# sMedX/FaceNet

Hardware: AMD Instinct MI355X
Metric: images/sec (160x160 triplet train) (higher is better)
Workload: dtype bf16

## Files before the change

### facenet_amd/_lib.py

```python
from __future__ import annotations

import ctypes as C
import os

import torch

_HERE = os.path.dirname(os.path.abspath(__file__))
LIB_PATH = os.path.join(_HERE, "lib", "libfacenet_hip.so")

FN_BF16, FN_F16 = 0, 1
FN_OPT_ADAGRAD, FN_OPT_ADADELTA, FN_OPT_RMSPROP, FN_OPT_MOM = 1, 2, 3, 4


class ConvDesc(C.Structure):
    _fields_ = [
        ("N", C.c_int32), ("H", C.c_int32), ("W", C.c_int32), ("Cin", C.c_int32),
        ("OH", C.c_int32), ("OW", C.c_int32), ("Cout", C.c_int32),
        ("KH", C.c_int32), ("KW", C.c_int32), ("stride", C.c_int32), ("pad_h", C.c_int32), ("pad_w", C.c_int32),
        ("dtype", C.c_int32), ("ld_x", C.c_int32), ("ld_y", C.c_int32),
        ("relu", C.c_int32), ("accumulate", C.c_int32), ("out_f32", C.c_int32), ("ld_res", C.c_int32),
        ("scale", C.c_float), ("splits", C.c_int32), ("stats_sq_off", C.c_int32), ("stats_replicas", C.c_int32),
        ("stats_rep_stride", C.c_int32),
        ("x", C.c_void_p), ("w", C.c_void_p), ("y", C.c_void_p), ("dx", C.c_void_p), ("dw", C.c_void_p),
        ("bias", C.c_void_p), ("stats", C.c_void_p), ("resid", C.c_void_p),
# ... 11 lines not shown

class FacenetHipError(RuntimeError):
    pass


_i, _f, _p, _l, _u = C.c_int, C.c_float, C.c_void_p, C.c_long, C.c_uint32

_SIGNATURES = {
    "fn_abi_version": [],
    "fn_conv2d_fwd": [C.POINTER(ConvDesc), _p],
    "fn_conv2d_dgrad": [C.POINTER(ConvDesc), _p],
    "fn_conv2d_wgrad": [C.POINTER(ConvDesc), _p],
    "fn_conv2d_variant": [C.POINTER(ConvDesc), _i],
    "fn_block35_infer": [_p, _p, _i, _p, _p, _p, _p, _p, _p, _f, _i, _i, _p],
    "fn_block35_infer_warm": [_p, _p, _i, _p, _p, _p, _p, _p, _p, _f, _i, _p, C.c_int64, _i, _p],
    "fn_block17_infer": [_p, _p, _i, _p, _p, _p, _p, _p, _p, _p, _p, _p, _p, _f, _i, _i, _p],
    "fn_block17_infer_warm": [_p, _p, _i, _p, _p, _p, _p, _p, _p, _p, _p, _p, _p, _f, _i, _p, C.c_int64, _i, _p],
    "fn_conv2d_arg_bytes": [],
    "fn_conv2d_group_build": [C.POINTER(ConvDesc), _i, _i, _i, _p, _p, _p],
    "fn_conv2d_grouped": [_p, _p, _i, _i, _i, _i, _i, _i, _p],
    "fn_conv2d_wgrad_arg_bytes": [],
    "fn_conv2d_wgrad_group_build": [C.POINTER(ConvDesc), _i, _i, _p, _p, _p, _p],
    "fn_conv2d_wgrad_reduce": [_p, _i, _p],
    "fn_conv2d_wgrad_grouped": [_p, _p, _i, _i, _i, _i, _p],
    "fn_image_normalize": [_p, _p, _p, _i, _i, _i, _i, _p],
    "fn_image_normalize_f32": [_p, _p, _p, _i, _i, _i, _i, _p],
    "fn_image_resize_bilinear": [_p, _i, _p, _i, _i, _i, _i, _i, _p],
    "fn_bn_finalize": [_p, _i, _i, _p, _p, _p, _p, _p, _p, _p, _f, _f, _i, _p],
    "fn_crop_or_pad_u8": [_p, _p, _p, _p, _i, _i, _p],
    "fn_augment_u8": [_p, _p, _p, _p, _p, _i, _i, _p],
    "fn_gather_images": [_p, _p, _p, _i, _i, _p],
    "fn_bn_relu_train_fwd": [_p, _i, _p, _i, _i, _i, _p, _i, _i, _i, _p, _p, _p, _p, _p, _f, _f, _i, _i, _p],
    "fn_bn_relu_train_bwd": [_p, _i, _p, _i, _i, _i, _p, _p, _p, _p, _p, _i, _i, _i, _i, _i, _i, _p],
    "fn_maxpool3x3s2_fwd": [_p, _i, _p, _i, _i, _i, _i, _i, _p, _i, _p],
    "fn_maxpool3x3s2_bwd": [_p, _i, _p, _i, _p, _i, _i, _i, _i, _i, _p, _i, _i, _p],
    "fn_area_resize_crop": [_p, _i, _i, _p, _i, _i, _i, _i, _p, _i, _p],
    "fn_maxpool2d_fwd": [_p, _i, _p, _i, _i, _i, _i, _i, _i, _i, _i, _i, _i, _i, _i, _p],
    "fn_area_resize_frame": [_p, _i, _i, _i, _i, _p, _p, _i, _p],
    "fn_mtcnn_candidates": [_p, C.c_long, _i, _f, _p, _p, _i, _i, _i, _p],
    "fn_nms_greedy_batch": [_p, _i, _p, _p, _p, _p, _i, _p, C.c_long, _p, _p, _p],
    "fn_nms_greedy": [_p, _i, _p, _i, C.c_double, _i, _p, C.c_long, _p, _p, _p],
    "fn_avgpool_fwd": [_p, _p, _i, _i, _i, _i, _p],
    "fn_avgpool_bwd": [_p, _p, _i, _i, _i, _i, _p],
    "fn_avgpool3x3s1_fwd": [_p, _i, _p, _i, _i, _i, _i, _i, _i, _p],
    "fn_avgpool3x3s1_bwd": [_p, _i, _p, _i, _i, _i, _i, _i, _i, _i, _p],
    "fn_dropout_fwd": [_p, _p, _i, _i, _f, _u, _i, _p, _i, _p],
    "fn_dropout_bwd": [_p, _p, _i, _i, _f, _u, _i, _p, _i, _p],
    "fn_residual_bwd": [_p, _p, _p, _p, _p, _i, _i, _f, _i, _i, _i, _p],
    "fn_acc_to_float": [_p, _p, _l, _i, _p],
    "fn_head_bn_fwd": [_p, _p, _i, _i, _p, _p, _p, _p, _p, _i, _f, _f, _p],
    "fn_head_bn_bwd": [_p, _p, _p, _p, _p, _p, _i, _i, _i, _p],
    "fn_l2norm_fwd": [_p, _p, _i, _i, _f, _p],
    "fn_l2norm_bwd": [_p, _p, _p, _i, _i, _f, _p],
    "fn_cast_f32_to_lp": [_p, _p, _l, _i, _p],
    "fn_pairwise_sqdist": [_p, _p, _p, _p, _i, _i, _i, _i, _p],
    "fn_select_triplets": [_p, _p, _i, _f, _i, _u, _i, _p, _p, _p],
    "fn_triplet_loss_fwd_bwd": [_p, _p, _p, _i, _i, _f, _p],
    "fn_confidence_counts": [_p, _p, _i, _i, _p, _i, _i, _p, _p, _p],
    "fn_confidence_counts_folds": [_p, _p, _p, _p, _p, _i, _i, _i, _p, _i, _i, _p, _p, _p],
    "fn_softmax_xent_fwd_bwd": [_p, _i, _p, _p, _p, _i, _p, _i, _i, _f, _i, _p],
    "fn_center_loss_fwd_bwd": [_p, _p, _p, _p, _p, _p, _i, _i, _i, _i, _f, _f, _f, _p],
    "fn_center_update": [_p, _i, _i, _i, _p, _i, C.c_double, _p],
    "fn_f2f_row_norms": [_p, _i, _i, _p, _p],
    "fn_f2f_pair_loss_fwd_bwd": [_p, _p, _i, _p, _i, _i, _i, _i, _f, _p, _p, _p, _p, _l, _p],
    "fn_f2f_pair_counts": [_p, _p, _p, _i, _i, _i, _p, _p, _p],
    "fn_f2f_distance": [_p, _p, _i, _p, _p, _i, _i, _i, _p, _i, _p, _p],
    "fn_adam_keras":[_p, _p, _p, _p, _p, _l, _l, _l, _p, _f, _f, _f, _f, _i, _p],
    "fn_adam_keras_ema": [_p, _p, _p, _p, _p, _l, _l, _l, _p, _f, _f, _f, _f, _i, _p, _f, _p],
    "fn_adam_tick": [_p, _f, _f, _p],
    "fn_opt_keras": [_i, _p, _p, _p, _p, _p, _l, _l, _l, _p, _f, _f, _f, _f, _i, _p],
    "fn_opt_keras_ema": [_i, _p, _p, _p, _p, _p, _l, _l, _l, _p, _f, _f, _f, _f, _i, _p, _f, _p],
    "fn_pack_transpose": [_p, _p, _p, _i, _i, _i, _p],
# ... 44 lines not shown
```

### facenet_amd/csrc/common.h

```cpp
#pragma once
#include <hip/hip_runtime.h>
#include <stdint.h>
#include <atomic>

namespace fn {

enum { FN_OK = 0, FN_EINVAL = -1, FN_ELAUNCH = -2, FN_EUNSUPPORTED = -3 };
void set_error(const char* fmt, ...);
int check_launch(const char* what);

#define FN_REQUIRE(cond, ...)                  \
    do {                                       \
        if (!(cond)) {                         \
            fn::set_error(__VA_ARGS__);        \
            return fn::FN_EINVAL;              \
        }                                      \
    } while (0)

typedef __attribute__((ext_vector_type(8))) __bf16 bf16x8;
typedef __attribute__((ext_vector_type(4))) __bf16 bf16x4;
typedef __attribute__((ext_vector_type(8))) _Float16 f16x8;
typedef __attribute__((ext_vector_type(4))) _Float16 f16x4;
typedef __attribute__((ext_vector_type(4))) float f32x4;
typedef __attribute__((ext_vector_type(4))) short s16x4;
// ... 90 lines not shown
    const float a = moving * momentum, w = 1.f - momentum;
    const float b = batch * w;
    return a + b;
}

__device__ __forceinline__ void bn_batch_affine(const acc_t* __restrict__ stats, int c, int sq_off, int reps, int rep_stride, int count,
                                                float eps, float beta, float& scale, float& shift, float& mean, float& var) {
    acc_t s = 0, q = 0;
    for (int rp = 0; rp < reps; ++rp) {
        s += stats[(long)rp * rep_stride + c];
        q += stats[(long)rp * rep_stride + sq_off + c];
    }
    bn_affine_from_sums(acc_get<ACC_STAT>(s), acc_get<ACC_STAT>(q), count, eps, beta, scale, shift, mean, var);
}

enum { STORE_WT = 17 };
__device__ __forceinline__ __amdgpu_buffer_rsrc_t wt_rsrc(const void* base) {
    return __builtin_amdgcn_make_buffer_rsrc(const_cast<void*>(base), 0, 0x7fffffff, 0x00020000);
}
__device__ __forceinline__ void store_wt(const __amdgpu_buffer_rsrc_t rs, long byte_offset, u32x4 v) {
    __builtin_amdgcn_raw_buffer_store_b128(v, rs, (int)byte_offset, 0, STORE_WT);
}

__device__ __forceinline__ int xcd_remap(int bid, int nwg) {
    const int q = nwg >> 3, r = nwg & 7, x = bid & 7;
    const int base = (x < r) ? x * (q + 1) : r * (q + 1) + (x - r) * q;
    return base + (bid >> 3);
}

static inline int cdiv(long a, long b) { return (int)((a + b - 1) / b); }

struct LdsOptIn {
    std::atomic<bool> done[32];
};
static inline int allow_big_lds(const void* kernel, LdsOptIn& state, const char* what) {
    int dev = 0;
    if (hipGetDevice(&dev) != hipSuccess || dev < 0 || dev >= 32) {
        set_error("%s: no current HIP device (or more than 32 devices)", what);
        return FN_ELAUNCH;
    }
    if (state.done[dev].load(std::memory_order_relaxed)) return FN_OK;
    const hipError_t e = hipFuncSetAttribute(kernel, hipFuncAttributeMaxDynamicSharedMemorySize, 160 * 1024);
    if (e != hipSuccess) {
        set_error("%s: hipFuncSetAttribute(MaxDynamicSharedMemorySize, 160 KiB) failed on device %d: %s", what, dev, hipGetErrorString(e));
        return FN_ELAUNCH;
    }
    state.done[dev].store(true, std::memory_order_relaxed);
// ... 12 lines not shown
```

### facenet_amd/csrc/conv_igemm.hip

```cpp
#include "common.h"
#include "../../include/facenet_hip.h"
#include "wgrad_taps.h"
#include <cstdio>
#include <type_traits>
#include <cstdlib>

#ifndef FN_IG_DBG
#define FN_IG_DBG 0
#endif

#if FN_IG_DBG & 32
__device__ unsigned long long fn_ig_phase[256 * 576 * 16];
extern "C" int fn_debug_phases(unsigned long long* out, int reset) {
    static unsigned long long host[256 * 576 * 16];
    if (out) {
        if (hipMemcpyFromSymbol(host, HIP_SYMBOL(fn_ig_phase), sizeof(host)) != hipSuccess) return -1;
        for (int i = 0; i < 576 * 16; ++i) {
            out[i] = 0;
            for (int r = 0; r < 256; ++r) out[i] += host[r * 576 * 16 + i];
        }
    }
    if (reset) {
        for (auto& v : host) v = 0;
        if (hipMemcpyToSymbol(HIP_SYMBOL(fn_ig_phase), host, sizeof(host)) != hipSuccess) return -1;
// ... 1173 lines not shown
    FN_REQUIRE(d->Cin % 8 == 0, "conv: Cin=%d must be a multiple of 8 (pad the input channels)", d->Cin);
    FN_REQUIRE(d->ld_x % 8 == 0 && d->ld_x >= d->Cin, "conv: ld_x=%d invalid for Cin=%d", d->ld_x, d->Cin);
    FN_REQUIRE(d->stride == 1 || d->stride == 2, "conv: stride %d unsupported", d->stride);
    FN_REQUIRE(d->KH >= 1 && d->KW >= 1 && d->KH < 256 && d->KW < 256, "conv: kernel %dx%d unsupported", d->KH, d->KW);
    FN_REQUIRE(d->N > 0 && d->H > 0 && d->W > 0 && d->OH > 0 && d->OW > 0 && d->Cout > 0, "conv: empty geometry");
    FN_REQUIRE((d->H + 2 * d->pad_h - d->KH) / d->stride + 1 == d->OH && (d->W + 2 * d->pad_w - d->KW) / d->stride + 1 == d->OW,
               "conv: OHxOW=%dx%d inconsistent with HxW=%dx%d k=%dx%d s=%d pad=%d,%d", d->OH, d->OW, d->H, d->W, d->KH, d->KW,
               d->stride, d->pad_h, d->pad_w);
    FN_REQUIRE((long)d->N * d->H * d->W < (1L << 31) / 8 && (long)d->N * d->OH * d->OW < (1L << 24) * 8L,
               "conv: tensor too large for 32-bit pixel indexing");
    return FN_OK;
}

struct WgradArgs {
    WgradOut out;
    const unsigned short* x;
    const unsigned short* dy;
    float* dw;
    int M, OH, OW, H, W, Cin, Cout, KTOT, KW;
    int stride, pad_h, pad_w;
    int ld_x, ld_y;
    int chunk;
    int gx, gy, splits;
    int plain;
    float inv_ow, inv_ohw;
    int x_bytes, dy_bytes;
    const acc_t* nrm_stats;
    const float* nrm_beta;
    int nrm_sq_off, nrm_replicas, nrm_rep_stride, nrm_count;
    float nrm_eps;
};

template <typename T, int BMW, int BNW, bool NORM>
__device__ __forceinline__ void conv_wgrad_body(const WgradArgs& a, const int bx, const int by, const int bz) {
    constexpr int BK = 64;
    constexpr int DEPTH = (BMW * BNW <= 64 * 64) ? 3 : (BMW * BNW <= 64 * 128 ? 2 : 1);
    constexpr int RSA = BMW * 2 + 32;
    constexpr int RSB = BNW * 2 + 32;
    constexpr int A_BYTES = BK * RSA, B_BYTES = BK * RSB;
    constexpr int CGA = BMW / 8, CGB = BNW / 8;
    constexpr int AP = BK * CGA / 256, BP = BK * CGB / 256;
    constexpr int WMW = (BMW >= 64) ? 2 : 1, WNW = 4 / WMW;
    constexpr int TM = BMW / WMW, TN = BNW / WNW;
    constexpr int MREP = TM / 16, NREP = TN / 16;
    static_assert(AP >= 1 && BP >= 1 && MREP >= 1 && NREP >= 1, "tile too small");
    typedef typename LP<T>::vec8 vec8;
// ... 185 lines not shown
    const long n4 = (long)a.Cout * a.KTOT / 4;
    const f32x4* ws = reinterpret_cast<const f32x4*>(a.ws);
    f32x4* dw = reinterpret_cast<f32x4*>(a.dw);
    for (long i = (long)blockIdx.x * 256 + threadIdx.x; i < n4; i += (long)gridDim.x * 256) {
        f32x4 s = ws[i];
        int z = 1;
        for (; z + 8 <= a.splits; z += 8) {
            f32x4 v[8];
#pragma unroll
            for (int k = 0; k < 8; ++k) v[k] = ws[(long)(z + k) * n4 + i];
#pragma unroll
            for (int k = 0; k < 8; ++k) s += v[k];
        }
        for (; z < a.splits; ++z) s += ws[(long)z * n4 + i];
        dw[i] = s;
    }
}

template <typename T, int BMW, int BNW, bool NORM>
__global__ __launch_bounds__(256) void conv_wgrad_kernel(const WgradArgs a) {
    conv_wgrad_body<T, BMW, BNW, NORM>(a, blockIdx.x, blockIdx.y, blockIdx.z);
}

template <typename T, int BMW, int BNW, bool NORM>
__global__ __launch_bounds__(256) void conv_wgrad_grouped_kernel(const unsigned char* __restrict__ args_raw, int stride, const int* __restrict__ prefix, int n) {
    const int bid = blockIdx.x;
    int lo = 0, hi = n;
    while (hi - lo > 1) {
        const int mid = (lo + hi) >> 1;
        if (prefix[mid] <= bid) lo = mid; else hi = mid;
    }
    lo = __builtin_amdgcn_readfirstlane(lo);
    const WgradArgs a = *reinterpret_cast<const WgradArgs*>(args_raw + (long)lo * stride);
    const int gxy = a.gx * a.gy;
    const int local = xcd_remap(bid - prefix[lo], gxy * a.splits);
    const int bz = local / gxy, r = local - bz * gxy;
    conv_wgrad_body<T, BMW, BNW, NORM>(a, r % a.gx, r / a.gx, bz);
}

template <typename T, int BMW, int BNW> static int launch_wgrad(const WgradArgs& a, int splits, hipStream_t st) {
    constexpr int RSA = BMW * 2 + 32, RSB = BNW * 2 + 32;
    const size_t smem = 2 * 64 * (RSA + RSB) + (a.nrm_stats ? 2 * BNW * 4 : 0);
    dim3 grid(cdiv(a.KTOT, BNW), cdiv(a.Cout, BMW), splits);
    if (a.nrm_stats) hipLaunchKernelGGL((conv_wgrad_kernel<T, BMW, BNW, true>), grid, dim3(256), smem, st, a);
    else hipLaunchKernelGGL((conv_wgrad_kernel<T, BMW, BNW, false>), grid, dim3(256), smem, st, a);
    return check_launch("conv_wgrad");
}

static void choose_wgrad_tile(int Cout, int KTOT, int& bmw, int& bnw) {
    bmw = Cout <= 32 ? 32 : (Cout <= 64 || Cout % 128 != 0 ? 64 : 128);
    bnw = (KTOT <= 64 || (cdiv(KTOT, 128) * 128 - KTOT) > 32) ? 64 : 128;
}

static int choose_wgrad_splits(int M, int Cout, int KTOT, int bmw, int bnw) {
    const long tiles = (long)cdiv(KTOT, bnw) * cdiv(Cout, bmw);
    const int stages = cdiv(M, 64);
    static const int stem_wgs = getenv("FN_WG_STEMWGS") ? atoi(getenv("FN_WG_STEMWGS")) : 1024;
    if (stages >= 1024) {
        int s = (int)((stem_wgs + tiles - 1) / tiles);
        if (s > stages / 4) s = stages / 4;
// ... 273 lines not shown
    long total = 0;
    for (int i = 0; i < n; ++i) {
        WgradArgs a;
        if (int rc = make_wgrad_args(&descs[i], a)) return rc;
        int m, k;
        final_wgrad_tile(a.Cout, a.KTOT, m, k);
        FN_REQUIRE(m == bmw && k == bnw, "wgrad_group_build: descriptor %d dispatches to %dx%d, group is %dx%d", i, m, k, bmw, bnw);
        FN_REQUIRE(descs[i].dtype == descs[0].dtype, "wgrad_group_build: mixed dtypes");
        FN_REQUIRE((a.nrm_stats != nullptr) == norm, "wgrad_group_build: descriptor %d: normalise-on-load members need a group of their own (variant + 1000000)", i);
        const int splits = plan_wgrad(a, descs[i].splits, bmw, bnw, true);
        FN_REQUIRE(((long)a.Cout * a.KTOT) % 4 == 0, "wgrad_group_build: descriptor %d: Cout*K must be a multiple of 4", i);
        a.out = WgradOut{a.dw, nullptr, a.Cout, a.KTOT, splits, 1};
        if (splits > 1) {
            a.out.ws = ws ? ws + ws_used : reinterpret_cast<float*>(16);
            ws_used += (long)splits * a.Cout * a.KTOT;
        }
        host_prefix[i] = (int32_t)total;
        total += (long)a.gx * a.gy * splits;
        *reinterpret_cast<WgradArgs*>(reinterpret_cast<unsigned char*>(host_args) + i * rec_bytes) = a;
    }
    FN_REQUIRE(total < (1L << 30), "wgrad_group_build: too many workgroups");
    host_prefix[n] = (int32_t)total;
    *ws_elems = ws_used;
    return (int)total;
}

extern "C" int fn_conv2d_wgrad_reduce(const void* dev_args, int n, void* stream) {
    FN_REQUIRE(dev_args && n > 0 && n < 65536, "wgrad_reduce: bad arguments");
    hipLaunchKernelGGL(wgrad_reduce_kernel, dim3(64, n), dim3(256), 0, (hipStream_t)stream, reinterpret_cast<const unsigned char*>(dev_args),
                       fn_conv2d_wgrad_arg_bytes());
    return check_launch("wgrad_reduce");
}

template <typename T> static int launch_wgrad_grouped(const void* args, const int32_t* prefix, int n, int total, int variant, hipStream_t st) {
    const bool norm = variant >= 1000000;
    variant %= 1000000;
    const int bmw = variant / 1000, bnw = variant % 1000;
    const unsigned char* a = reinterpret_cast<const unsigned char*>(args);
    const int stride_ = fn_conv2d_wgrad_arg_bytes();
#define FN_WG(BM_, BN_)                                                                                                     \
    if (bmw == BM_ && bnw == BN_) {                                                                                         \
        const size_t sm_ = 2 * 64 * ((BM_) * 2 + 32 + (BN_) * 2 + 32) + (norm ? 2 * (BN_) * 4 : 0);                            \
        if (norm) hipLaunchKernelGGL((conv_wgrad_grouped_kernel<T, BM_, BN_, true>), dim3(total), dim3(256), sm_, st, a, stride_, prefix, n); \
        else hipLaunchKernelGGL((conv_wgrad_grouped_kernel<T, BM_, BN_, false>), dim3(total), dim3(256), sm_, st, a, stride_, prefix, n);    \
        return check_launch("conv_wgrad_grouped");                                                                          \
    }
    FN_WG(32, 64) FN_WG(32, 128) FN_WG(64, 64) FN_WG(64, 128) FN_WG(128, 64) FN_WG(128, 128)
// ... 35 lines not shown
```

### facenet_amd/csrc/elementwise.hip

```cpp
#include "common.h"
#include "../../include/facenet_hip.h"

namespace fn {

__device__ __forceinline__ unsigned f2ord(float f) {
    unsigned u = __float_as_uint(f);
    return (u & 0x80000000u) ? ~u : (u | 0x80000000u);
}
__device__ __forceinline__ float ord2f(unsigned u) {
    return __uint_as_float((u & 0x80000000u) ? (u & 0x7fffffffu) : ~u);
}

template <typename SRC>
__global__ __launch_bounds__(256) void img_stats_kernel(const SRC* __restrict__ img, unsigned* __restrict__ work, int count) {
    const int n = blockIdx.y;
    const SRC* p = img + (long)n * count;
    float mx = -3e38f, mn = 3e38f, s = 0.f, q = 0.f;
    constexpr int PER = 16 / sizeof(SRC);
    const int head = min(count, (int)(((16 - ((uintptr_t)p & 15)) & 15) / sizeof(SRC)));
    const int nvec = (count - head) / PER;
    const SRC* pv = p + head;
    for (int i = blockIdx.x * 256 + threadIdx.x; i < nvec; i += gridDim.x * 256) {
        const u32x4 v = *reinterpret_cast<const u32x4*>(pv + (long)i * PER);
#pragma unroll
// ... 968 lines not shown
extern "C" int fn_l2norm_bwd(const float* x, const float* dout, float* dx, int N, int E, float eps, void* stream) {
    FN_REQUIRE(x && dout && dx && N > 0 && E > 0, "l2norm_bwd: bad arguments");
    hipLaunchKernelGGL(l2norm_bwd_kernel, dim3(cdiv(N, 4)), dim3(256), 0, (hipStream_t)stream, x, dout, dx, N, E, eps);
    return check_launch("l2norm_bwd");
}
extern "C" int fn_cast_f32_to_lp(const float* x, void* y, long n, int dtype, void* stream) {
    DT_CHECK(dtype);
    FN_REQUIRE(x && y && n > 0, "cast: bad arguments");
    LAUNCH_T(dtype, cast_kernel, dim3(grid_for(n)), dim3(256), 0, (hipStream_t)stream, x, (unsigned short*)y, n);
    return check_launch("cast");
}

namespace fn {
__global__ __launch_bounds__(256) void acc_to_float_kernel(const acc_t* __restrict__ src, float* __restrict__ dst, long n, double scale) {
    for (long i = (long)blockIdx.x * 256 + threadIdx.x; i < n; i += (long)gridDim.x * 256) dst[i] = (float)((double)src[i] * scale);
}
}
extern "C" int fn_acc_to_float(const fn_acc_t* src, float* dst, long n, int bits, void* stream) {
    FN_REQUIRE(src && dst && n > 0 && bits >= 0 && bits < 63, "acc_to_float: bad arguments");
    hipLaunchKernelGGL(acc_to_float_kernel, dim3(grid_for(n)), dim3(256), 0, (hipStream_t)stream, reinterpret_cast<const acc_t*>(src), dst, n,
                       1.0 / (double)(1ll << bits));
    return check_launch("acc_to_float");
}
```

### facenet_amd/train.py

```python
from __future__ import annotations

import contextlib
import ctypes as C
import json
import os
import warnings
from typing import Callable, Dict, List, NamedTuple, Optional, Sequence, Tuple

import numpy as np
import torch

from . import _lib, parallel
from .config import Config
from .engine import BN_EPS, L2_WEIGHT, Lowering, Network, _pad8, _ptr
from .schedule import Op, Schedule, StreamSet, levelize, make_events, region, run_schedule, torch_op


class GraphRunner:

    def __init__(self, device: torch.device):
        self.device = device
        self.graphs: List[torch.cuda.CUDAGraph] = []
        self.pool = None

    def capture(self, fn: Callable[[], None]) -> torch.cuda.CUDAGraph:
        g = torch.cuda.CUDAGraph()
        with torch.cuda.graph(g, pool=self.pool):
            fn()
        if self.pool is None:
            self.pool = g.pool()
        self.graphs.append(g)
        return g


def group_wgrads(ops: List[Op], net: Network) -> List[Op]:
    lib = net.lib
    singles = [op for op in ops if op.name.startswith("conv_wgrad:") and op.keep]
    if len(singles) < 2:
        return list(ops)
    rest = [op for op in ops if not (op.name.startswith("conv_wgrad:") and op.keep)]
    groups = {}
    for op in singles:
        d = op.keep[0]
        v = lib.fn_conv2d_variant(C.byref(d), 2)
        groups.setdefault((v + (1000000 if d.nrm_stats and v < 5000000 else 0), d.dtype), []).append(op)
    nbytes = lib.fn_conv2d_wgrad_arg_bytes()
    out = list(rest)
    split_tables, split_keep, split_writes = [], [], []
    for (variant, dt), members in sorted(groups.items()):
        n = len(members)
        descs = (_lib.ConvDesc * n)(*[m.keep[0] for m in members])
        host_args = (C.c_uint8 * (nbytes * n))()
        host_prefix = (C.c_int32 * (n + 1))()
        ws_elems = C.c_int64(0)
        total = lib.fn_conv2d_wgrad_group_build(descs, n, variant, host_args, host_prefix, None, C.byref(ws_elems))
        if total < 0:
            _lib.check(total, "wgrad_group_build")
        ws = torch.empty(max(1, ws_elems.value), dtype=torch.float32, device=net.device)
        total = lib.fn_conv2d_wgrad_group_build(descs, n, variant, host_args, host_prefix, _ptr(ws), C.byref(ws_elems))
        if total < 0:
            _lib.check(total, "wgrad_group_build")
        dev_args = torch.frombuffer(bytearray(host_args), dtype=torch.uint8).to(net.device)
        dev_prefix = torch.tensor(list(host_prefix), dtype=torch.int32, device=net.device)
        reads, writes = [], []
        for m in members:
            reads.extend(m.reads)
            writes.extend(m.writes)
        if variant >= 5000000:
            code = variant - 5000000
            name = f"conv_wgrad_taps:{code // 1000}x{code % 1000 // 10}" + ("s2" if code % 10 else "")
        else:
            name = f"conv_wgrad_grouped:{variant % 1000000 // 1000}x{variant % 1000}" + (":norm" if variant >= 1000000 else "")
# ... 230 lines not shown
        self.G = net.alloc_grads()
        self.slots: List[torch.Tensor] = [torch.full_like(self.G, init) for _, init in self.rule.slots]
        self.M, self.V = self.slots if self.optimizer == "ADAM" else (None, None)
        self.hyper = torch.tensor([lr, 1.0, 1.0, 1.0 / world_size, 0.0, 0.0, 0.0, 0.0], dtype=torch.float32, device=dev)
        self.loss = torch.zeros(4, dtype=torch.float32, device=dev)
        if world_size > 1:
            parallel.broadcast_parameters([net.P, net.S_mean, net.S_var], src=0, group=process_group)
            net.folded_valid = False
            net.refresh_packs()
        self.shadow: Optional[torch.Tensor] = None if self.ema_decay is None else net.P.clone()
        rank = 0
        if self.exchange:
            import torch.distributed as dist
            rank = dist.get_rank(process_group)
        self.rank = rank
        self.plan: Lowering = net.plan(batch, training=True, step_word=self.hyper.view(torch.int32)[4:5], rank=rank)
        self.demb = torch.zeros(batch, E, dtype=torch.float32, device=dev)
        self.dt = _lib.dtype_code(net.train_dtype)
        ebuf = self.plan.embedding.buf
        emb = ebuf.act
        r_emb = region(emb)
        self.emb = emb.view(batch, E)
        self.pre_ops: List[Op] = [
            Op("zero_grads", torch_op(lambda: (self.G.zero_(), net.Gacc.zero_())), (), writes=(region(self.G), region(net.Gacc))),
            Op("zero_bn_workspace", torch_op(lambda: (self.plan.ws.zero_(), self.plan.ws_b.zero_())), (),
               writes=(region(self.plan.ws), (self.plan.ws.data_ptr() + 1, 0, net.CB), region(self.plan.ws_b),
                       (self.plan.ws_b.data_ptr() + 1, 0, net.CB))),
        ]
        self.loss_ops: List[Op] = []
        if loss == "triplet":
            self.embn = torch.zeros(batch, E, dtype=torch.float32, device=dev)
            self.dembn = torch.zeros(batch, E, dtype=torch.float32, device=dev)
            self._op(self.loss_ops, "l2norm_fwd", lib.fn_l2norm_fwd, _ptr(emb), _ptr(self.embn), batch, E, 1e-10,
                     r=[r_emb], w=[region(self.embn)])
            self._op(self.loss_ops, "triplet_loss", lib.fn_triplet_loss_fwd_bwd, _ptr(self.embn), _ptr(self.dembn), _ptr(self.loss),
                     batch // 3, E, alpha, r=[region(self.embn)], w=[region(self.dembn), region(self.loss)])
            self._op(self.loss_ops, "l2norm_bwd", lib.fn_l2norm_bwd, _ptr(emb), _ptr(self.dembn), _ptr(self.demb), batch, E, 1e-10,
                     r=[r_emb, region(self.dembn)], w=[region(self.demb)])
        else:
            L = net.layers["classifier/logits"]
            Cp, Cr = L.cout, L.cout_real
            self.labels = torch.zeros(batch, dtype=torch.int32, device=dev)
            self.emb_lp = torch.zeros(batch, E, dtype=net.train_dtype, device=dev)
            self.logits = torch.zeros(batch, Cp, dtype=torch.float32, device=dev)
            self.dlogits = torch.zeros(batch, Cp, dtype=net.train_dtype, device=dev)
            rw = region(net.W_train, L.w_off, L.w_off + L.numel)
            rwt = region(net.Wt_train, L.w_off, L.w_off + L.numel)
            rgw = region(self.G, L.w_off, L.w_off + L.numel)
            rgb = region(net.Gacc, L.bias_off - net.bias_lo, L.bias_off - net.bias_lo + L.cout)
            d = self._cls_desc(L)
# ... 25 lines not shown
                        net.n_decay, _ptr(self.hyper), beta1, beta2, epsilon, l2, self.dt)
        else:
            rule = self.rule
            name, fn, fn_ema = rule.op, lib.fn_opt_keras, lib.fn_opt_keras_ema
            s2 = _ptr(self.slots[1]) if len(self.slots) > 1 else None
            opt_args = (rule.code, _ptr(net.P), _ptr(self.G), _ptr(self.slots[0]), s2, _ptr(net.W_train), net.n_kernel, net.n_params,
                        net.n_decay, _ptr(self.hyper), rule.rho, rule.momentum, rule.epsilon, l2, self.dt)
        if self.shadow is None:
            self._op(self.opt_ops, name, fn, *opt_args, r=[region(self.G), region(self.hyper)], w=opt_writes)
        else:
            self._op(self.opt_ops, name + "_ema", fn_ema, *opt_args, _ptr(self.shadow), self.ema_decay,
                     r=[region(self.G), region(self.hyper)], w=opt_writes + [region(self.shadow)])
        self._op(self.opt_ops, "pack_transpose", lib.fn_pack_transpose, _ptr(net.W_train), _ptr(net.Wt_train), _ptr(net.table),
                 len(net.layers), net.max_layer_elems, self.dt, r=[region(net.W_train)], w=[region(net.Wt_train)])
        if self.centers is not None:
            self._op(self.opt_ops, "center_update", lib.fn_center_update, _ptr(self.center_rows), E + 1, self.world * batch, E,
                     _ptr(self.centers), self.centers.shape[0], self.center_alfa, r=[region(self.center_rows)], w=[region(self.centers)])
        n_buckets = int(os.environ.get("FACENET_DP_BUCKETS", n_buckets))
        self.buckets = self._make_buckets(n_buckets) if self.segmented else []
        self.comm_stream = torch.cuda.Stream(device=dev) if self.exchange else None
        self.streams = _streams_for(net, n_streams)
        self.tiles = autotune_convs(self.plan.fwd + self.loss_ops + self.plan.bwd, net)
        self._build_segments()
        self._graph = None
        self._exchange_events: Optional[dict] = None
        self._eval_plans: Dict[int, Tuple[Lowering, torch.Tensor]] = {}
        self._average_in_place = False

    def _op(self, lst, name, fn, *args, keep=(), r=(), w=()):
        lst.append(Op(name, fn, args, tuple(keep), tuple(r), tuple(w)))

    def _build_regularizers(self, n_classes: int, rank: int, r_emb):
        net, lib, N, E, dev = self.net, self.net.lib, self.N, self.net.E, self.net.device
        self.reg_terms = torch.zeros(8, dtype=torch.float32, device=dev)
        reads, writes = [r_emb, region(self.labels), region(self.demb)], [region(self.demb), region(self.reg_terms)]
        rows, slot = None, None
        if self.center_factor > 0:
            self.centers = torch.zeros(n_classes, E, dtype=torch.float32, device=dev)
            self.center_rows = torch.zeros(self.world, N, E + 1, dtype=torch.float32, device=dev)
            rows, slot = self.center_rows[rank], region(self.center_rows, rank * N * (E + 1), (rank + 1) * N * (E + 1))
            reads.append(region(self.centers))
            writes.append(slot)
            if self.world > 1:
                self.pre_ops.append(Op("zero_center_rows", torch_op(lambda: self.center_rows.zero_()), (),
                                       writes=(region(self.center_rows),)))
        self._op(self.loss_ops, "center_loss", lib.fn_center_loss_fwd_bwd, _ptr(self.emb), _ptr(self.labels),
# ... 32 lines not shown
            if chunks > 0 and self.group_wgrad:
                marks = [i for i, op in enumerate(self.plan.bwd) if op.name.startswith("conv_wgrad:")]
                cuts = [0] + [marks[len(marks) * k // chunks] for k in range(1, chunks)] + [len(self.plan.bwd)]
                ops: List[Op] = []
                for k in range(chunks):
                    ops += grp((head if k == 0 else []) + self.plan.bwd[cuts[k]:cuts[k + 1]])
                ops += self.opt_ops
                for op in ops:
                    op.stream_hint = 1 if op.name.startswith("conv_wgrad") else 0
                self.n_streams = max(2, self.n_streams)
                self.streams = _streams_for(self.net, self.n_streams)
                self.segments.append((Schedule(ops, self.n_streams), None))
                return
            self.segments.append((Schedule(grp(head + self.plan.bwd) + self.opt_ops, self.n_streams), None))
            return
        pos, first = 0, True
        for (ready, lo, hi) in self.buckets:
            a, b = pos, max(pos, ready)
            ops = grp((head if first else []) + self.plan.bwd[a:b])
            self.segments.append((Schedule(ops, self.n_streams) if ops else None, (lo, hi)))
            pos, first = b, False
        assert pos == len(self.plan.bwd)
        self.segments.append((Schedule(self.opt_ops, 1), None))

    @property
    def step_ops(self) -> List[Op]:
        out: List[Op] = []
        for sched, _ in self.segments:
            if sched is not None:
                out.extend(sched.ops)
        return out

    def _zero(self):
        self.G.zero_()
        self.net.Gacc.zero_()
        self.plan.ws.zero_()
        self.plan.ws_b.zero_()

    def _run_segments(self, launch: Callable[[int], None]):
        self.net.folded_valid = False
        if not self.segmented:
            launch(0)
            return
        if not self.exchange:
            for i, (sched, _) in enumerate(self.segments):
                if sched is not None:
# ... 343 lines not shown
```

### include/facenet_hip.h

```cpp
#ifndef FACENET_HIP_H
#define FACENET_HIP_H
#include <stdint.h>
#ifdef __cplusplus
extern "C" {
#endif

#define FN_BF16 0
#define FN_F16 1

typedef int64_t fn_acc_t;
#define FN_ACC_STAT_BITS 20
#define FN_ACC_GRAD_BITS 40

const char* fn_last_error(void);
int fn_abi_version(void);

typedef struct fn_conv_desc {
    int32_t N, H, W, Cin;
    int32_t OH, OW, Cout;
    int32_t KH, KW, stride, pad_h, pad_w;
    int32_t dtype;
    int32_t ld_x, ld_y;
    int32_t relu;
    int32_t accumulate;
// ... 42 lines not shown
int fn_block17_infer(const void* x, void* y, int N, const void* w_t0, const void* w_t1a, const void* w_t1b, const void* w_t1c, const void* w_up,
                     const float* b_t0, const float* b_t1a, const float* b_t1b, const float* b_t1c, const float* b_up, float scale, int relu,
                     int dtype, void* stream);
int fn_block17_infer_warm(const void* x, void* y, int N, const void* w_t0, const void* w_t1a, const void* w_t1b, const void* w_t1c,
                          const void* w_up, const float* b_t0, const float* b_t1a, const float* b_t1b, const float* b_t1c, const float* b_up,
                          float scale, int relu, const void* warm, int64_t warm_bytes, int dtype, void* stream);
int fn_block35_infer(const void* x, void* y, int N, const void* const* w_1x1, const void* const* w_3x3, const void* w_up,
                     const float* const* b_1x1, const float* const* b_3x3, const float* b_up, float scale, int relu, int dtype, void* stream);
int fn_block35_infer_warm(const void* x, void* y, int N, const void* const* w_1x1, const void* const* w_3x3, const void* w_up,
                          const float* const* b_1x1, const float* const* b_3x3, const float* b_up, float scale, int relu,
                          const void* warm, int64_t warm_bytes, int dtype, void* stream);
int fn_conv2d_fwd(const fn_conv_desc* d, void* stream);
int fn_conv2d_dgrad(const fn_conv_desc* d, void* stream);
int fn_conv2d_wgrad(const fn_conv_desc* d, void* stream);
int fn_conv2d_arg_bytes(void);
int fn_conv2d_group_build(const fn_conv_desc* descs, int n, int op, int variant, void* host_args, int32_t* host_prefix, int32_t* smem_bytes);
int fn_conv2d_grouped(const void* dev_args, const int32_t* dev_prefix, int n, int total_blocks, int variant, int plain, int smem_bytes,
                      int dtype, void* stream);
int fn_conv2d_wgrad_arg_bytes(void);
int fn_conv2d_wgrad_group_build(const fn_conv_desc* descs, int n, int variant, void* host_args, int32_t* host_prefix, float* ws,
                                int64_t* ws_elems);
int fn_conv2d_wgrad_grouped(const void* dev_args, const int32_t* dev_prefix, int n, int total_blocks, int variant, int dtype, void* stream);
int fn_conv2d_wgrad_reduce(const void* dev_args, int n, void* stream);
int fn_conv2d_variant(const fn_conv_desc* d, int op);

int fn_image_normalize(const uint8_t* img, void* out, float* work, int N, int HW, int mode, int dtype, void* stream);
int fn_image_normalize_f32(const float* img, void* out, float* work, int N, int HW, int mode, int dtype, void* stream);
int fn_image_resize_bilinear(const void* img, int src_is_f32, float* out, int N, int H, int W, int OH, int OW, void* stream);
int fn_crop_or_pad_u8(const uint8_t* src, const long long* offsets, const int32_t* hw, uint8_t* dst, int N, int S, void* stream);
typedef struct fn_augment_param {
    int32_t y0, x0;
    int32_t flip;
    float cos_t, sin_t;
} fn_augment_param;
int fn_augment_u8(const uint8_t* src, const long long* offsets, const int32_t* hw, const fn_augment_param* params, uint8_t* dst, int N,
                  int S, void* stream);
int fn_gather_images(const uint8_t* pool, const int32_t* idx, uint8_t* out, int n_out, int bytes_per_image, void* stream);

int fn_bn_finalize(const fn_acc_t* stats, int sq_off, int rep_stride, const int32_t* reps, const int32_t* count, const float* beta,
                   float* save_scale, float* save_shift, float* moving_mean, float* moving_var, float momentum, float eps, int CB,
                   void* stream);

int fn_bn_relu_train_fwd(const void* y, int ld_y, void* z, int ld_z, int M, int C, const fn_acc_t* stats, int stats_sq_off, int stats_replicas,
                         int stats_rep_stride, const float* beta,
                         float* save_scale, float* save_shift, float* moving_mean, float* moving_var, float momentum, float eps,
                         int relu, int dtype, void* stream);
// ... 7 lines not shown
int fn_area_resize_crop(const uint8_t* frame, int H, int W, const int32_t* boxes, int n, int OH, int OW, int source_is_u8, void* out,
                        int dtype, void* stream);
int fn_maxpool2d_fwd(const void* x, int ld_x, void* y, int ld_y, int N, int H, int W, int C, int k, int stride, int pad_h, int pad_w,
                     int OH, int OW, int dtype, void* stream);
int fn_area_resize_frame(const uint8_t* frame, int H, int W, int OH, int OW, float* rows, void* out, int dtype, void* stream);
int fn_mtcnn_candidates(const float* map, long ncell, int ld, float threshold, float* cand, int32_t* counter, int max_cand, int tag,
                        int reset_counter, void* stream);
int fn_nms_greedy(const double* boxes, int ld, const int32_t* order, int n, double threshold, int by_min, void* workspace,
                  long workspace_bytes, int32_t* keep, int32_t* n_keep, void* stream);
int fn_nms_greedy_batch(const double* boxes, int ld, const int32_t* order, const int32_t* sizes, const double* thresholds, const int32_t* by_min,
                        int njobs, void* workspace, long workspace_bytes, int32_t* keep, int32_t* n_keep, void* stream);
int fn_avgpool_fwd(const void* x, void* y, int N, int HW, int C, int dtype, void* stream);
int fn_avgpool_bwd(const void* dy, void* dx, int N, int HW, int C, int dtype, void* stream);
int fn_avgpool3x3s1_fwd(const void* x, int ld_x, void* y, int ld_y, int N, int H, int W, int C, int dtype, void* stream);
int fn_avgpool3x3s1_bwd(const void* dy, int ld_dy, void* dx, int ld_dx, int N, int H, int W, int C, int accumulate, int dtype,
                        void* stream);
int fn_dropout_fwd(const void* x, void* y, int N, int C, float keep, unsigned seed, int rank, const int32_t* step, int dtype, void* stream);
int fn_dropout_bwd(const void* dy, void* dx, int N, int C, float keep, unsigned seed, int rank, const int32_t* step, int dtype, void* stream);

int fn_residual_bwd(const void* dout, const void* out, void* dtrunk, void* dup, fn_acc_t* dbias, int M, int C, float scale, int relu,
                    int accumulate, int dtype, void* stream);

int fn_acc_to_float(const fn_acc_t* src, float* dst, long n, int bits, void* stream);

int fn_head_bn_fwd(const float* y, float* out, int N, int E, const float* beta, float* moving_mean, float* moving_var,
                   float* save_mean, float* save_rstd, int training, float momentum, float eps, void* stream);
int fn_head_bn_bwd(const float* dout, const float* y, const float* save_mean, const float* save_rstd, float* dbeta, void* dy_lp,
                   int N, int E, int dtype, void* stream);
int fn_l2norm_fwd(const float* x, float* out, int N, int E, float eps, void* stream);
int fn_l2norm_bwd(const float* x, const float* dout, float* dx, int N, int E, float eps, void* stream);
int fn_cast_f32_to_lp(const float* x, void* y, long n, int dtype, void* stream);

int fn_pairwise_sqdist(const float* xa, const float* xb, float* out, float* range, int n, int m, int E, int metric, void* stream);
int fn_select_triplets(const float* dist, const int32_t* labels, int n, float alpha, int nrof_triplets, uint32_t seed,
                       int semi_hard, int32_t* triplets, int32_t* info, void* stream);
int fn_triplet_loss_fwd_bwd(const float* emb, float* demb, float* loss, int T, int E, float alpha, void* stream);

int fn_confidence_counts(const float* emb, const int32_t* cls_start, int C, int E, const float* thresholds, int T, int metric,
                         double* out, int32_t* range, void* stream);

int fn_confidence_counts_folds(const float* emb, const int32_t* cls_start, const int32_t* fold, const int32_t* train_rows,
                               const int32_t* train_classes, int C, int E, int F, const float* thresholds, int T, int metric,
                               double* out, int32_t* range, void* stream);

int fn_softmax_xent_fwd_bwd(const float* logits, int ld, const int32_t* labels, float* loss, void* dlogits_lp, int ld_d, fn_acc_t* dbias, int N,
                            int C, float grad_scale, int dtype, void* stream);
// ... 36 lines not shown
```

Before: 13890.

## Zero only accumulated gradient ranges and co-schedule sibling wgrads sharing input

Replaces the per-step zeroing of the full gradient buffer and BN workspaces with one fused fill kernel. That kernel clears only the gradient ranges written by accumulating ops plus the accumulator and workspace buffers. Ranges written by storing ops are skipped, and padding is zeroed once at setup. Grouped wgrad members that read the same input activation are sorted together and share one XCD remap space, so tiles reading the same x land on the same XCD for cache reuse. The risk is a stale gradient if an op is wrongly classified as storing.

Result: no change. 13930 (median of 3 runs) (+0.3%).

```diff
diff --git a/facenet_amd/_lib.py b/facenet_amd/_lib.py
--- a/facenet_amd/_lib.py
+++ b/facenet_amd/_lib.py
@@ -57,6 +57,7 @@
     "fn_conv2d_wgrad_arg_bytes": [],
     "fn_conv2d_wgrad_group_build": [C.POINTER(ConvDesc), _i, _i, _p, _p, _p, _p],
     "fn_conv2d_wgrad_reduce": [_p, _i, _p],
+    "fn_conv2d_wgrad_group_locate": [_p, _p, _i, _i, _p],
     "fn_conv2d_wgrad_grouped": [_p, _p, _i, _i, _i, _i, _p],
     "fn_image_normalize": [_p, _p, _p, _i, _i, _i, _i, _p],
     "fn_image_normalize_f32": [_p, _p, _p, _i, _i, _i, _i, _p],
@@ -83,6 +84,7 @@
     "fn_dropout_bwd": [_p, _p, _i, _i, _f, _u, _i, _p, _i, _p],
     "fn_residual_bwd": [_p, _p, _p, _p, _p, _i, _i, _f, _i, _i, _i, _p],
     "fn_acc_to_float": [_p, _p, _l, _i, _p],
+    "fn_fill_ranges": [_p, _i, _p],
     "fn_head_bn_fwd": [_p, _p, _i, _i, _p, _p, _p, _p, _p, _i, _f, _f, _p],
     "fn_head_bn_bwd": [_p, _p, _p, _p, _p, _p, _i, _i, _i, _p],
     "fn_l2norm_fwd": [_p, _p, _i, _i, _f, _p],
diff --git a/facenet_amd/csrc/common.h b/facenet_amd/csrc/common.h
--- a/facenet_amd/csrc/common.h
+++ b/facenet_amd/csrc/common.h
@@ -136,7 +136,7 @@
     __builtin_amdgcn_raw_buffer_store_b128(v, rs, (int)byte_offset, 0, STORE_WT);
 }
 
-__device__ __forceinline__ int xcd_remap(int bid, int nwg) {
+__host__ __device__ __forceinline__ int xcd_remap(int bid, int nwg) {
     const int q = nwg >> 3, r = nwg & 7, x = bid & 7;
     const int base = (x < r) ? x * (q + 1) : r * (q + 1) + (x - r) * q;
     return base + (bid >> 3);
diff --git a/facenet_amd/csrc/conv_igemm.hip b/facenet_amd/csrc/conv_igemm.hip
--- a/facenet_amd/csrc/conv_igemm.hip
+++ b/facenet_amd/csrc/conv_igemm.hip
@@ -1219,6 +1219,10 @@
     int ld_x, ld_y;
     int chunk;
     int gx, gy, splits;
+    int fam_lead;
+    int fam_n;
+    int fam_gxy;
+    int fam_toff;
     int plain;
     float inv_ow, inv_ohw;
     int x_bytes, dy_bytes;
@@ -1450,20 +1454,38 @@
     conv_wgrad_body<T, BMW, BNW, NORM>(a, blockIdx.x, blockIdx.y, blockIdx.z);
 }
 
-template <typename T, int BMW, int BNW, bool NORM>
-__global__ __launch_bounds__(256) void conv_wgrad_grouped_kernel(const unsigned char* __restrict__ args_raw, int stride, const int* __restrict__ prefix, int n) {
-    const int bid = blockIdx.x;
+__host__ __device__ inline int wgrad_group_locate(const unsigned char* __restrict__ args_raw, int stride, const int* __restrict__ prefix,
+                                                  int n, int bid, int& bx, int& by, int& bz) {
     int lo = 0, hi = n;
     while (hi - lo > 1) {
         const int mid = (lo + hi) >> 1;
         if (prefix[mid] <= bid) lo = mid; else hi = mid;
     }
+#if defined(__HIP_DEVICE_COMPILE__)
     lo = __builtin_amdgcn_readfirstlane(lo);
-    const WgradArgs a = *reinterpret_cast<const WgradArgs*>(args_raw + (long)lo * stride);
-    const int gxy = a.gx * a.gy;
-    const int local = xcd_remap(bid - prefix[lo], gxy * a.splits);
-    const int bz = local / gxy, r = local - bz * gxy;
-    conv_wgrad_body<T, BMW, BNW, NORM>(a, r % a.gx, r / a.gx, bz);
+#endif
+    const WgradArgs* rec = reinterpret_cast<const WgradArgs*>(args_raw + (long)lo * stride);
+    const int first = lo - rec->fam_lead, members = rec->fam_n, gxy = rec->fam_gxy;
+    const int local = xcd_remap(bid - prefix[first], gxy * rec->splits);
+    bz = local / gxy;
+    const int r = local - bz * gxy;
+    int m = first, toff = 0;
+    for (int k = 1; k < members; ++k) {
+        const int t = reinterpret_cast<const WgradArgs*>(args_raw + (long)(first + k) * stride)->fam_toff;
+        if (r >= t) { m = first + k; toff = t; }
+    }
+    const int gx = reinterpret_cast<const WgradArgs*>(args_raw + (long)m * stride)->gx;
+    bx = (r - toff) % gx;
+    by = (r - toff) / gx;
+    return m;
+}
+
+template <typename T, int BMW, int BNW, bool NORM>
+__global__ __launch_bounds__(256) void conv_wgrad_grouped_kernel(const unsigned char* __restrict__ args_raw, int stride, const int* __restrict__ prefix, int n) {
+    int bx, by, bz;
+    const int m = wgrad_group_locate(args_raw, stride, prefix, n, blockIdx.x, bx, by, bz);
+    const WgradArgs a = *reinterpret_cast<const WgradArgs*>(args_raw + (long)m * stride);
+    conv_wgrad_body<T, BMW, BNW, NORM>(a, bx, by, bz);
 }
 
 template <typename T, int BMW, int BNW> static int launch_wgrad(const WgradArgs& a, int splits, hipStream_t st) {
@@ -1783,7 +1805,35 @@
     FN_REQUIRE(total < (1L << 30), "wgrad_group_build: too many workgroups");
     host_prefix[n] = (int32_t)total;
     *ws_elems = ws_used;
+    auto rec_at = [&](int i) { return reinterpret_cast<WgradArgs*>(reinterpret_cast<unsigned char*>(host_args) + i * rec_bytes); };
+    auto siblings = [](const WgradArgs& p, const WgradArgs& q) {
+        return p.x == q.x && p.ld_x == q.ld_x && p.x_bytes == q.x_bytes && p.M == q.M && p.OH == q.OH && p.OW == q.OW && p.H == q.H &&
+               p.W == q.W && p.Cin == q.Cin && p.KTOT == q.KTOT && p.KW == q.KW && p.stride == q.stride && p.pad_h == q.pad_h &&
+               p.pad_w == q.pad_w && p.chunk == q.chunk && p.splits == q.splits && p.nrm_stats == q.nrm_stats && p.nrm_beta == q.nrm_beta;
+    };
+    for (int i = 0; i < n;) {
+        int j = i + 1;
+        while (j < n && siblings(*rec_at(i), *rec_at(j))) ++j;
+        int gxy = 0;
+        for (int k = i; k < j; ++k) {
+            rec_at(k)->fam_lead = k - i;
+            rec_at(k)->fam_n = j - i;
+            rec_at(k)->fam_toff = gxy;
+            gxy += rec_at(k)->gx * rec_at(k)->gy;
+        }
+        for (int k = i; k < j; ++k) rec_at(k)->fam_gxy = gxy;
+        i = j;
+    }
     return (int)total;
+}
+
+extern "C" int fn_conv2d_wgrad_group_locate(const void* host_args, const int32_t* host_prefix, int n, int bid, int32_t* out) {
+    FN_REQUIRE(host_args && host_prefix && out && n > 0, "wgrad_group_locate: bad arguments");
+    FN_REQUIRE(bid >= 0 && bid < host_prefix[n], "wgrad_group_locate: workgroup %d outside the group's %d", bid, host_prefix[n]);
+    int bx, by, bz;
+    out[0] = wgrad_group_locate(reinterpret_cast<const unsigned char*>(host_args), fn_conv2d_wgrad_arg_bytes(), host_prefix, n, bid, bx, by, bz);
+    out[1] = bz; out[2] = bx; out[3] = by;
+    return FN_OK;
 }
 
 extern "C" int fn_conv2d_wgrad_reduce(const void* dev_args, int n, void* stream) {
diff --git a/facenet_amd/csrc/elementwise.hip b/facenet_amd/csrc/elementwise.hip
--- a/facenet_amd/csrc/elementwise.hip
+++ b/facenet_amd/csrc/elementwise.hip
@@ -1014,3 +1014,28 @@
                        1.0 / (double)(1ll << bits));
     return check_launch("acc_to_float");
 }
+
+namespace fn {
+struct FillRange {
+    unsigned* p;
+    long n;
+};
+__global__ __launch_bounds__(256) void fill_ranges_kernel(const FillRange* __restrict__ table) {
+    const FillRange a = table[blockIdx.y];
+    long head = (long)((0 - (reinterpret_cast<uintptr_t>(a.p) >> 2)) & 3);
+    if (head > a.n) head = a.n;
+    u32x4* const v = reinterpret_cast<u32x4*>(a.p + head);
+    const long nv = (a.n - head) >> 2, done = head + nv * 4;
+    const u32x4 z = {0u, 0u, 0u, 0u};
+    for (long i = (long)blockIdx.x * 256 + threadIdx.x; i < nv; i += (long)gridDim.x * 256) v[i] = z;
+    if (blockIdx.x == 0) {
+        if (threadIdx.x < head) a.p[threadIdx.x] = 0u;
+        if (threadIdx.x < a.n - done) a.p[done + threadIdx.x] = 0u;
+    }
+}
+}
+extern "C" int fn_fill_ranges(const void* dev_table, int n, void* stream) {
+    FN_REQUIRE(dev_table && n > 0 && n < 65536, "fill_ranges: bad arguments");
+    hipLaunchKernelGGL(fill_ranges_kernel, dim3(64, n), dim3(256), 0, (hipStream_t)stream, reinterpret_cast<const FillRange*>(dev_table));
+    return check_launch("fill_ranges");
+}
diff --git a/facenet_amd/train.py b/facenet_amd/train.py
--- a/facenet_amd/train.py
+++ b/facenet_amd/train.py
@@ -31,6 +31,37 @@
             self.pool = g.pool()
         self.graphs.append(g)
         return g
+
+
+_STORES_GRADS = ("conv_wgrad_grouped", "conv_wgrad_taps", "conv_wgrad_reduce", "grad_finalize")
+
+
+def _merge_ranges(rs: Sequence[Tuple[int, int]]) -> List[Tuple[int, int]]:
+    out: List[Tuple[int, int]] = []
+    for lo, hi in sorted(rs):
+        if out and lo <= out[-1][1]:
+            out[-1] = (out[-1][0], max(out[-1][1], hi))
+        else:
+            out.append((lo, hi))
+    return out
+
+
+def _subtract_ranges(rs: Sequence[Tuple[int, int]], cut: Sequence[Tuple[int, int]]) -> List[Tuple[int, int]]:
+    out: List[Tuple[int, int]] = []
+    for lo, hi in rs:
+        for c_lo, c_hi in cut:
+            if c_hi <= lo or c_lo >= hi:
+                continue
+            if c_lo > lo:
+                out.append((lo, c_lo))
+            lo = max(lo, c_hi)
+        if lo < hi:
+            out.append((lo, hi))
+    return out
+
+
+def _wgrad_source(d) -> tuple:
+    return (d.x, d.ld_x, d.N, d.H, d.W, d.Cin, d.OH, d.OW, d.KH, d.KW, d.stride, d.pad_h, d.pad_w, d.splits, d.nrm_stats)
 
 
 def group_wgrads(ops: List[Op], net: Network) -> List[Op]:
@@ -48,6 +79,10 @@
     out = list(rest)
     split_tables, split_keep, split_writes = [], [], []
     for (variant, dt), members in sorted(groups.items()):
+        first: Dict[tuple, int] = {}
+        for i, m in enumerate(members):
+            first.setdefault(_wgrad_source(m.keep[0]), i)
+        members.sort(key=lambda m: first[_wgrad_source(m.keep[0])])
         n = len(members)
         descs = (_lib.ConvDesc * n)(*[m.keep[0] for m in members])
         host_args = (C.c_uint8 * (nbytes * n))()
@@ -324,10 +359,9 @@
         r_emb = region(emb)
         self.emb = emb.view(batch, E)
         self.pre_ops: List[Op] = [
-            Op("zero_grads", torch_op(lambda: (self.G.zero_(), net.Gacc.zero_())), (), writes=(region(self.G), region(net.Gacc))),
-            Op("zero_bn_workspace", torch_op(lambda: (self.plan.ws.zero_(), self.plan.ws_b.zero_())), (),
-               writes=(region(self.plan.ws), (self.plan.ws.data_ptr() + 1, 0, net.CB), region(self.plan.ws_b),
-                       (self.plan.ws_b.data_ptr() + 1, 0, net.CB))),
+            Op("zero_step_state", lib.fn_fill_ranges, (None, 0),
+               writes=(region(self.G), region(net.Gacc), region(self.plan.ws), (self.plan.ws.data_ptr() + 1, 0, net.CB),
+                       region(self.plan.ws_b), (self.plan.ws_b.data_ptr() + 1, 0, net.CB))),
         ]
         self.loss_ops: List[Op] = []
         if loss == "triplet":
@@ -399,6 +433,7 @@
         self.streams = _streams_for(net, n_streams)
         self.tiles = autotune_convs(self.plan.fwd + self.loss_ops + self.plan.bwd, net)
         self._build_segments()
+        self._plan_zeroing()
         self._graph = None
         self._exchange_events: Optional[dict] = None
         self._eval_plans: Dict[int, Tuple[Lowering, torch.Tensor]] = {}
@@ -477,6 +512,29 @@
             pos, first = b, False
         assert pos == len(self.plan.bwd)
         self.segments.append((Schedule(self.opt_ops, 1), None))
+
+    def _plan_zeroing(self):
+        G, zero = self.G, self.pre_ops[0]
+        ops = self.step_ops
+        assert any(op is zero for op in ops), "the step lost its zero_step_state launch"
+        stored, accumulated = [], []
+        for op in ops:
+            if op is zero:
+                continue
+            for base, lo, hi in op.writes:
+                if base == G.data_ptr() and hi > lo:
+                    (stored if op.name.split(":")[0] in _STORES_GRADS else accumulated).append((lo, hi))
+        accumulated = _merge_ranges(accumulated)
+        stored = _subtract_ranges(_merge_ranges(stored), accumulated)
+        padding = _subtract_ranges([(0, G.numel())], _merge_ranges(stored + accumulated))
+        self.grad_ranges = {"stored": stored, "accumulated": accumulated, "padding": padding}
+        for lo, hi in padding:
+            G[lo:hi].zero_()
+        ws, ws_b, Gacc = self.plan.ws, self.plan.ws_b, self.net.Gacc
+        rows = [(_ptr(G, lo), hi - lo) for lo, hi in accumulated]
+        rows += [(_ptr(t), t.numel() * t.element_size() // 4) for t in (Gacc, ws, ws_b)]
+        self._zero_table = torch.tensor(rows, dtype=torch.int64, device=G.device)
+        zero.args = (_ptr(self._zero_table), len(rows))
 
     @property
     def step_ops(self) -> List[Op]:
diff --git a/include/facenet_hip.h b/include/facenet_hip.h
--- a/include/facenet_hip.h
+++ b/include/facenet_hip.h
@@ -88,6 +88,7 @@
                                 int64_t* ws_elems);
 int fn_conv2d_wgrad_grouped(const void* dev_args, const int32_t* dev_prefix, int n, int total_blocks, int variant, int dtype, void* stream);
 int fn_conv2d_wgrad_reduce(const void* dev_args, int n, void* stream);
+int fn_conv2d_wgrad_group_locate(const void* host_args, const int32_t* host_prefix, int n, int bid, int32_t* out);
 int fn_conv2d_variant(const fn_conv_desc* d, int op);
 
 int fn_image_normalize(const uint8_t* img, void* out, float* work, int N, int HW, int mode, int dtype, void* stream);
@@ -141,6 +142,7 @@
                     int accumulate, int dtype, void* stream);
 
 int fn_acc_to_float(const fn_acc_t* src, float* dst, long n, int bits, void* stream);
+int fn_fill_ranges(const void* dev_table, int n, void* stream);
 
 int fn_head_bn_fwd(const float* y, float* out, int N, int E, const float* beta, float* moving_mean, float* moving_var,
                    float* save_mean, float* save_rstd, int training, float momentum, float eps, void* stream);
```
